# opendilab/LightZero

Measured on NVIDIA H100. Metric: MCTS simulations/sec (batched search+infer), higher is better.
Workload: dtype f32 (fp16x2-split tensor MMAs, fp32 accumulate)

## Files before the change

lightzero_b200/csrc/conv_tc.cu:

```cuda
#include <math.h>
#include <stdlib.h>
#include <string.h>

#include <algorithm>

#include "conv_tc.cuh"
#include "tc_ptx.cuh"

namespace lz {

constexpr int kCvConsumers = 256, kCvThreads = kCvConsumers + 32;
constexpr int kCvStages = 4;

struct CvBars {
    uint64_t full[kCvStages], empty[kCvStages];
    uint64_t in_full;
};

struct CvGeom {
    int nbands, rin, m_lo, mcount, NT, PR;
    size_t plane, part, phase, in_bytes, tap_bytes, smem;
};

__host__ __device__ inline CvGeom cv_geom(const ConvTc &p)
// ... 106 lines not shown
                wg_wait<1>();
                __syncwarp();
                if (lane == 0) mbar_arrive(&bars->empty[(n - 1) % nstages]);
            }
        }
        wg_wait<0>();
        __syncwarp();
        if (lane == 0) mbar_arrive(&bars->empty[(t * 9 + 8) % nstages]);

#pragma unroll
        for (int hr = 0; hr < 2; ++hr) {
            const int m = g.m_lo + t * 128 + wg * 64 + 16 * (warp & 3) + (lane >> 2) + 8 * hr;
            const int k = m / g.rin;
            const int rho = rin0 + (m - k * g.rin);
            const int yy = rho / pitch - 1, xx = rho - (yy + 1) * pitch;
            const bool in_band = (k < nimg) && (rho >= pitch) && (yy >= y0) && (yy < yend);
            const bool valid = in_band && (xx < W);
#pragma unroll
            for (int j = 0; j < N / 8; ++j) {
                const int col = 8 * j + qc;
                const int grp = (N == 128) ? (col >> 6) : 0;
                const int c = col - grp * 64;
                const Tcl &o = p.out[grp];
                const bool relu = p.relu[grp] != 0;
                float v0 = fmaf(acc[4 * j + 2 * hr], __ldg(p.scale + col), __ldg(p.shift + col));
                float v1 = fmaf(acc[4 * j + 2 * hr + 1], __ldg(p.scale + col + 1), __ldg(p.shift + col + 1));
                if (p.res.base && grp == 0 && valid) {
                    const unsigned char *rp = p.res.base + (size_t)(img0 + k) * p.res.img_stride +
                                              ((size_t)(c >> 3) * p.res.plane_rows + rho + 1) * 16 + (c & 7) * 2;
                    const float2 a = __half22float2(*reinterpret_cast<const __half2 *>(rp));
                    const float2 b = __half22float2(*reinterpret_cast<const __half2 *>(rp + p.res.part_stride));
                    v0 += a.x + b.x;
                    v1 += a.y + b.y;
                }
                v0 = valid ? (relu ? fmaxf(v0, 0.0f) : v0) : 0.0f;
                v1 = valid ? (relu ? fmaxf(v1, 0.0f) : v1) : 0.0f;
                if (in_band) {
                    unsigned char *op = o.base + (size_t)(img0 + k) * o.img_stride + ((size_t)(c >> 3) * o.plane_rows + rho + 1) * 16 + (c & 7) * 2;
                    store_split2(op, op + o.part_stride, v0, v1);
                }
            }
        }
    }
}

constexpr int kRbChunks = 16;

struct RbBars {
    uint64_t full[kCvStages], empty[kCvStages];
    uint64_t chunk[kRbChunks];
};

struct RbGeom {
    int nbands, S, m_lo, NT1, NT2, PR, nchunk;
    size_t plane, part, buf, tap_bytes, smem;
};

__host__ __device__ inline RbGeom rb_geom(const ResBlockTc &p)
{
    RbGeom g;
    const int H = p.in.H, pitch = p.in.pitch, kg = p.in.C / 8;
    g.nbands = (H + p.band_h - 1) / p.band_h;
    g.S = (p.band_h + 4) * pitch + 2;
    g.m_lo = pitch + 1;
    g.NT1 = ((p.G - 1) * g.S + (p.band_h + 2) * pitch + 127) / 128;
    g.NT2 = ((p.G - 1) * g.S + p.band_h * pitch + 127) / 128;
    g.PR = p.G * g.S;
    g.nchunk = (g.PR + 127) / 128;
    g.plane = (size_t)g.PR * 16;
    g.part = (size_t)kg * g.plane;
    g.buf = (2 * g.part + 127) & ~(size_t)127;
    g.tap_bytes = (size_t)2 * kg * p.in.C * 16;
    g.smem = 2 * g.buf + p.stages * g.tap_bytes + 1024;
    return g;
}

template <int N>
__device__ __forceinline__ void rb_tiles(float (&acc)[2][N / 2], bool two, uint64_t a_desc0, int row0, const ResBlockTc &p,
                                         const RbGeom &g, uint64_t b_desc0, RbBars *bars, int n0, int lane)
{
    const uint32_t plane16 = (uint32_t)(g.plane >> 4), a_lo16 = (uint32_t)(g.part >> 4), b_lo16 = (uint32_t)N;
    const int nstages = p.stages;
#pragma unroll
    for (int s = 0; s < 2; ++s)
#pragma unroll
        for (int i = 0; i < N / 2; ++i) acc[s][i] = 0.0f;
    for (int tap = 0; tap < 9; ++tap) {
        const int n = n0 + tap, st = n % nstages;
        mbar_wait(&bars->full[st], (n / nstages) & 1);
        const uint64_t b0 = b_desc0 + (uint64_t)((st * g.tap_bytes) >> 4);
        const uint64_t a0 = a_desc0 + (uint64_t)(row0 + p.tap_shift[tap]);
        wg_fence();
        for (int ks = 0; ks < N / 16; ++ks) {
#pragma unroll
            for (int s = 0; s < 2; ++s) {
                if (s == 1 && !two) break;
                const uint64_t as = a0 + s * 128 + ks * 2 * plane16;
                wgmma_f16<N>(acc[s], as, b0 + ks * 4 * N);
                if (p.npass == 3) {
                    wgmma_f16<N>(acc[s], as, b0 + b_lo16 + ks * 4 * N);
                    wgmma_f16<N>(acc[s], as + a_lo16, b0 + ks * 4 * N);
                }
            }
        }
        wg_commit();
        if (tap > 0) {
            wg_wait<1>();
            __syncwarp();
            if (lane == 0) mbar_arrive(&bars->empty[(n - 1) % nstages]);
        }
    }
    wg_wait<0>();
    __syncwarp();
    if (lane == 0) mbar_arrive(&bars->empty[(n0 + 8) % nstages]);
}

template <int N>
__global__ void __launch_bounds__(kCvThreads, 1) k_resblock_tc(ResBlockTc p)
{
    extern __shared__ __align__(1024) unsigned char smem[];
    const RbGeom g = rb_geom(p);
    unsigned char *in_s = smem, *mid_s = smem + g.buf, *ring = smem + 2 * g.buf;
    RbBars *bars = reinterpret_cast<RbBars *>(ring + p.stages * g.tap_bytes);
    const int nstages = p.stages;
    const int tid = threadIdx.x, warp = __shfl_sync(0xffffffffu, tid >> 5, 0), lane = tid & 31;
    const int pitch = p.in.pitch, H = p.in.H, W = p.in.W, kg_in = N / 8;
    const int group = blockIdx.x / g.nbands, band = blockIdx.x - group * g.nbands;
    const int img0 = group * p.G, nimg = min(p.G, p.B - img0);
    const int y0 = band * p.band_h;
    const int np1 = (g.NT1 + 1) / 2, ntaps = 9 * (np1 + (g.NT2 + 1) / 2);

    if (tid == 0) {
        for (int i = 0; i < kCvStages; ++i) { mbar_init(&bars->full[i], 1); mbar_init(&bars->empty[i], kCvConsumers / 32); }
        for (int c = 0; c < g.nchunk; ++c) mbar_init(&bars->chunk[c], 1);
        fence_mbar_init();
    }
    __syncthreads();

    if (warp == kCvConsumers / 32) {
        if (lane == 0) {
            auto load_tap = [&](int n) {
                const int st = n % nstages, tap = n % 9;
                if (n >= nstages) mbar_wait(&bars->empty[st], ((n / nstages) - 1) & 1);
                mbar_expect_tx(&bars->full[st], (uint32_t)g.tap_bytes);
                bulk_g2s(ring + st * g.tap_bytes, p.w[n >= 9 * np1] + (size_t)tap * g.tap_bytes, (uint32_t)g.tap_bytes, &bars->full[st]);
            };
            for (int n = 0; n < nstages; ++n) load_tap(n);
            const int g0 = (y0 - 1) * pitch;
            const int r0 = max(0, -g0), r1 = min(g.S, p.in.plane_rows - g0);
            for (int c = 0; c < g.nchunk; ++c) {
                uint32_t rows = 0;
                for (int k = 0; k < nimg; ++k) rows += (uint32_t)max(0, min(k * g.S + r1, c * 128 + 128) - max(k * g.S + r0, c * 128));
                mbar_expect_tx(&bars->chunk[c], rows * 16u * (uint32_t)(2 * kg_in));
                for (int k = 0; k < nimg; ++k) {
                    const int lo = max(k * g.S + r0, c * 128), hi = min(k * g.S + r1, c * 128 + 128);
                    if (hi <= lo) continue;
                    for (int part = 0; part < 2; ++part)
                        for (int kg = 0; kg < kg_in; ++kg) {
                            const unsigned char *src = p.in.base + (size_t)(img0 + k) * p.in.img_stride + part * p.in.part_stride +
                                                       ((size_t)kg * p.in.plane_rows + g0 + lo - k * g.S) * 16;
                            bulk_g2s(in_s + part * g.part + kg * g.plane + (size_t)lo * 16, src, (uint32_t)(hi - lo) * 16u, &bars->chunk[c]);
                        }
                }
            }
            for (int n = nstages; n < ntaps; ++n) load_tap(n);
        }
        return;
    }

    const int wg = warp >> 2;
    const uint32_t plane16 = (uint32_t)(g.plane >> 4);
    const uint64_t in_desc = make_desc(smem_u32(in_s), plane16, 8), mid_desc = make_desc(smem_u32(mid_s), plane16, 8);
    const uint64_t b_desc0 = make_desc(smem_u32(ring), 2 * N, 8);
    const int qc = 2 * (lane & 3);
    if (tid < 2 * kg_in) *reinterpret_cast<uint4 *>(mid_s + tid * g.plane) = make_uint4(0u, 0u, 0u, 0u);

    int ready = 0;
    for (int t = 0; t < g.NT1; t += 2) {
        const bool two = t + 1 < g.NT1;
        const int need = min(g.nchunk, (t * 128 + 256 + 2 * pitch + 1) / 128 + 1);
        for (; ready < need; ++ready) mbar_wait(&bars->chunk[ready], 0);
        float acc[2][N / 2];
        rb_tiles<N>(acc, two, in_desc, g.m_lo + t * 128 + wg * 64, p, g, b_desc0, bars, t / 2 * 9, lane);
#pragma unroll
        for (int e = 0; e < 4; ++e) {
            const int s = e >> 1, hr = e & 1;
            if (s == 1 && !two) break;
            const int m = g.m_lo + (t + s) * 128 + wg * 64 + 16 * (warp & 3) + (lane >> 2) + 8 * hr;
            const int i = m - pitch;
            const int k = m / g.S;
            const int rho = (y0 - 1) * pitch - 1 + (m - k * g.S);
            const int yy = rho / pitch - 1, xx = rho - (yy + 1) * pitch;
            const bool valid = (k < nimg) && (rho >= pitch) && (yy >= y0 - 1) && (yy <= y0 + p.band_h) && (yy < H) && (xx < W);
            if (i >= g.PR) continue;
#pragma unroll
            for (int j = 0; j < N / 8; ++j) {
                const int col = 8 * j + qc;
                float v0 = fmaf(acc[s][4 * j + 2 * hr], __ldg(p.scale[0] + col), __ldg(p.shift[0] + col));
                float v1 = fmaf(acc[s][4 * j + 2 * hr + 1], __ldg(p.scale[0] + col + 1), __ldg(p.shift[0] + col + 1));
                v0 = valid ? fmaxf(v0, 0.0f) : 0.0f;
                v1 = valid ? fmaxf(v1, 0.0f) : 0.0f;
                unsigned char *op = mid_s + (size_t)(col >> 3) * g.plane + (size_t)i * 16 + (col & 7) * 2;
                store_split2(op, op + g.part, v0, v1);
            }
        }
    }
    for (; ready < g.nchunk; ++ready) mbar_wait(&bars->chunk[ready], 0);
    fence_proxy_async();
    asm volatile("bar.sync 1, %0;\n" ::"n"(kCvConsumers) : "memory");

    const int yend = min(y0 + p.band_h, H);
    for (int t = 0; t < g.NT2; t += 2) {
        const bool two = t + 1 < g.NT2;
        float acc[2][N / 2];
        rb_tiles<N>(acc, two, mid_desc, g.m_lo + t * 128 + wg * 64, p, g, b_desc0, bars, (np1 + t / 2) * 9, lane);
#pragma unroll
        for (int e = 0; e < 4; ++e) {
            const int s = e >> 1, hr = e & 1;
            if (s == 1 && !two) break;
            const int m = g.m_lo + (t + s) * 128 + wg * 64 + 16 * (warp & 3) + (lane >> 2) + 8 * hr;
            const int k = m / g.S;
            const int rho = y0 * pitch - 1 + (m - k * g.S);
            const int yy = rho / pitch - 1, xx = rho - (yy + 1) * pitch;
            const bool in_band = (k < nimg) && (rho >= pitch) && (yy >= y0) && (yy < yend);
            const bool valid = in_band && (xx < W);
            const Tcl &o = p.out;
            size_t obase = 0;
            bool do_write = in_band;
            if (in_band) {
                if (o.nphase == 1) {
                    obase = (size_t)(img0 + k) * o.img_stride + (size_t)(rho + 1) * 16;
                } else if (valid) {
                    const int ph = (yy & 1) * 2 + (xx & 1);
                    const int rho2 = ((yy >> 1) + 1) * o.pitch + (xx >> 1);
                    obase = (size_t)(img0 + k) * o.img_stride + ph * o.phase_stride + (size_t)(rho2 + 1) * 16;
                } else {
                    do_write = false;
                }
            }
#pragma unroll
            for (int j = 0; j < N / 8; ++j) {
                const int col = 8 * j + qc;
                float v0 = fmaf(acc[s][4 * j + 2 * hr], __ldg(p.scale[1] + col), __ldg(p.shift[1] + col));
                float v1 = fmaf(acc[s][4 * j + 2 * hr + 1], __ldg(p.scale[1] + col + 1), __ldg(p.shift[1] + col + 1));
                if (valid) {
                    const unsigned char *rp = in_s + (size_t)(col >> 3) * g.plane + (size_t)(m + pitch) * 16 + (col & 7) * 2;
                    const float2 a = __half22float2(*reinterpret_cast<const __half2 *>(rp));
                    const float2 b = __half22float2(*reinterpret_cast<const __half2 *>(rp + g.part));
                    v0 += a.x + b.x;
                    v1 += a.y + b.y;
                }
                v0 = valid ? fmaxf(v0, 0.0f) : 0.0f;
                v1 = valid ? fmaxf(v1, 0.0f) : 0.0f;
                if (do_write) {
                    unsigned char *op = o.base + obase + (size_t)(col >> 3) * o.plane_rows * 16 + (col & 7) * 2;
                    store_split2(op, op + o.part_stride, v0, v1);
                }
            }
        }
    }
}

__device__ __forceinline__ void tcl_load8(const Tcl &t, int img, int kg, int rho, float (&v)[8])
{
    const unsigned char *pp = t.base + (size_t)img * t.img_stride + ((size_t)kg * t.plane_rows + rho + 1) * 16;
    const uint4 rh = __ldg(reinterpret_cast<const uint4 *>(pp));
    const uint4 rl = __ldg(reinterpret_cast<const uint4 *>(pp + t.part_stride));
    const __half2 *hh = reinterpret_cast<const __half2 *>(&rh), *hl = reinterpret_cast<const __half2 *>(&rl);
#pragma unroll
    for (int j = 0; j < 4; ++j) {
        const float2 a = __half22float2(hh[j]), b = __half22float2(hl[j]);
        v[2 * j] = a.x + b.x;
        v[2 * j + 1] = a.y + b.y;
    }
}

__global__ void k_pool_tcl(Tcl in, Tcl out, float *out_nchw, int B, int Hout)
{
    const int kgs = in.C / 8;
    const size_t n = (size_t)B * kgs * Hout * Hout;
    for (size_t i = blockIdx.x * (size_t)blockDim.x + threadIdx.x; i < n; i += (size_t)gridDim.x * blockDim.x) {
        const int xo = (int)(i % Hout), yo = (int)((i / Hout) % Hout);
        const int kg = (int)((i / ((size_t)Hout * Hout)) % kgs), img = (int)(i / ((size_t)Hout * Hout * kgs));
        float s[8];
#pragma unroll
        for (int j = 0; j < 8; ++j) s[j] = 0.0f;
#pragma unroll
        for (int ky = 0; ky < 3; ++ky) {
            const int yy = 2 * yo + ky - 1;
            if (yy < 0 || yy >= in.H) continue;
#pragma unroll
            for (int kx = 0; kx < 3; ++kx) {
                const int xx = 2 * xo + kx - 1;
                if (xx < 0 || xx >= in.W) continue;
                float v[8];
                tcl_load8(in, img, kg, (yy + 1) * in.pitch + xx, v);
#pragma unroll
                for (int j = 0; j < 8; ++j) s[j] += v[j];
            }
        }
#pragma unroll
        for (int j = 0; j < 8; ++j) s[j] = s[j] / 9.0f;
        if (out_nchw) {
#pragma unroll
            for (int j = 0; j < 8; ++j) out_nchw[((size_t)img * in.C + kg * 8 + j) * Hout * Hout + yo * Hout + xo] = s[j];
        } else {
            unsigned char *op = out.base + (size_t)img * out.img_stride + ((size_t)kg * out.plane_rows + (yo + 1) * out.pitch + xo + 1) * 16;
            store_split8(op, op + out.part_stride, s);
        }
    }
}

int conv_tc_prepare_launch()
{
    const int big = 227 * 1024;
    LZ_CUDA_CHECK(cudaFuncSetAttribute(k_conv_tc<64>, cudaFuncAttributeMaxDynamicSharedMemorySize, big));
    LZ_CUDA_CHECK(cudaFuncSetAttribute(k_conv_tc<128>, cudaFuncAttributeMaxDynamicSharedMemorySize, big));
    LZ_CUDA_CHECK(cudaFuncSetAttribute(k_resblock_tc<32>, cudaFuncAttributeMaxDynamicSharedMemorySize, big));
    LZ_CUDA_CHECK(cudaFuncSetAttribute(k_resblock_tc<64>, cudaFuncAttributeMaxDynamicSharedMemorySize, big));
    return LZ_OK;
}

int conv_tc_launch(const ConvTc &p, cudaStream_t s)
{
    const CvGeom g = cv_geom(p);
    LZ_REQUIRE(g.smem <= 227 * 1024, LZ_EINVAL, "conv_tc: band needs %zu B shared memory", g.smem);
    LZ_REQUIRE(g.tap_bytes <= 16384 && (p.in.C % 16) == 0, LZ_EINVAL, "conv_tc: unsupported channel counts");
    LZ_REQUIRE(p.out[0].nphase == 1 && (p.N < 128 || p.out[1].nphase == 1), LZ_EINVAL, "conv_tc: phase-split output is not supported");
    const int groups = (p.B + p.G - 1) / p.G;
    const int grid = groups * g.nbands;
    switch (p.N) {
        case 64: k_conv_tc<64><<<grid, kCvThreads, g.smem, s>>>(p); break;
        case 128: k_conv_tc<128><<<grid, kCvThreads, g.smem, s>>>(p); break;
        default: LZ_REQUIRE(false, LZ_EINVAL, "conv_tc: N must be 64 or 128");
    }
    LZ_KERNEL_CHECK();
    return LZ_OK;
}

int resblock_tc_plan(ResBlockTc &p)
{
    const int H = p.in.H, W = p.in.W;
    ResBlockTc q = p;
    double best = -1.0;
    for (int G = 1; G <= 4; ++G)
        for (int bh = (G > 1 ? H : 1); bh <= H; ++bh)
            for (int st = 2; st <= 4; st += 2) {
                q.G = G; q.band_h = bh; q.stages = st;
                const RbGeom g = rb_geom(q);
                if (g.smem > 227 * 1024 || g.nchunk > kRbChunks) continue;
                double score = (double)(2 * G * H * W) / ((double)g.nbands * (g.NT1 + g.NT2) * 128);
                score *= (st == 4) ? 1.0 : 0.97;
                if (score > best + 1e-9) { best = score; p.G = G; p.band_h = bh; p.stages = st; }
            }
    LZ_REQUIRE(best > 0.0, LZ_EINVAL, "resblock_tc: no band of a %dx%d, %d-channel block fits shared memory", H, W, p.in.C);
    return LZ_OK;
}

int resblock_tc_launch(const ResBlockTc &p, cudaStream_t s)
{
    const RbGeom g = rb_geom(p);
    LZ_REQUIRE(g.smem <= 227 * 1024 && g.nchunk <= kRbChunks, LZ_EINVAL, "resblock_tc: band needs %zu B shared memory", g.smem);
    LZ_REQUIRE(p.in.nphase == 1 && p.out.C == p.in.C, LZ_EINVAL, "resblock_tc: unsupported input / output layout");
    const int grid = (p.B + p.G - 1) / p.G * g.nbands;
    switch (p.in.C) {
        case 32: k_resblock_tc<32><<<grid, kCvThreads, g.smem, s>>>(p); break;
        case 64: k_resblock_tc<64><<<grid, kCvThreads, g.smem, s>>>(p); break;
        default: LZ_REQUIRE(false, LZ_EINVAL, "resblock_tc: channels must be 32 or 64");
    }
    LZ_KERNEL_CHECK();
    return LZ_OK;
}

size_t conv_tc_packed_bytes(int cin, int ncols) { return (size_t)9 * 2 * (cin / 8) * ncols * 16; }

float conv_tc_pack(const float *w, int cin, int cout, int ncols, int col0, unsigned char *dst)
{
    float mx = 0.0f;
    for (size_t i = 0; i < (size_t)cout * cin * 9; ++i) mx = std::max(mx, fabsf(w[i]));
    int e = 0;
    if (mx > 0.0f) frexpf(mx, &e);
    const float scale = ldexpf(1.0f, 13 - e);
    const size_t tap_halves = (size_t)2 * (cin / 8) * ncols * 8, part_halves = (size_t)ncols * 8;
    __half *h = reinterpret_cast<__half *>(dst);
    for (int t = 0; t < 9; ++t)
        for (int co = 0; co < cout; ++co)
            for (int ci = 0; ci < cin; ++ci) {
                const float sv = w[((size_t)co * cin + ci) * 9 + t] * scale;
                const __half hi = __float2half_rn(sv);
                const __half lo = __float2half_rn(sv - __half2float(hi));
                const size_t off = (size_t)t * tap_halves + ((size_t)(ci / 8) * 2 * ncols + col0 + co) * 8 + (ci % 8);
                h[off] = hi;
                h[off + part_halves] = lo;
            }
    return scale;
}

int pool_tcl_launch(const Tcl &in, const Tcl &out, int B, cudaStream_t s)
{
    const size_t n = (size_t)B * (in.C / 8) * out.H * out.W;
    k_pool_tcl<<<(int)std::min<size_t>((n + 255) / 256, kNumSMs * 32), 256, 0, s>>>(in, out, nullptr, B, out.H);
    LZ_KERNEL_CHECK();
    return LZ_OK;
}

int pool_tcl_to_nchw_launch(const Tcl &in, float *out, int B, int Hout, cudaStream_t s)
{
    const size_t n = (size_t)B * (in.C / 8) * Hout * Hout;
    Tcl dummy = in;
    k_pool_tcl<<<(int)std::min<size_t>((n + 255) / 256, kNumSMs * 32), 256, 0, s>>>(in, dummy, out, B, Hout);
    LZ_KERNEL_CHECK();
    return LZ_OK;
}

}
```

lightzero_b200/csrc/conv_tc.cuh:

```cuda
#pragma once
#include "lz_common.cuh"

namespace lz {

struct Tcl {
    unsigned char *base;
    size_t img_stride, phase_stride, part_stride;
    int plane_rows;
    int C, H, W, pitch;
    int nphase;
};

inline Tcl make_tcl(unsigned char *base, int C, int H, int W, int nphase)
{
    Tcl t;
    t.base = base; t.C = C; t.H = H; t.W = W; t.pitch = W + 1; t.nphase = nphase;
    t.plane_rows = (H + 2) * (W + 1) + 2;
    t.part_stride = (size_t)(C / 8) * t.plane_rows * 16;
    t.phase_stride = 2 * t.part_stride;
    t.img_stride = t.phase_stride * nphase;
    return t;
}
inline size_t tcl_bytes(int B, int C, int H, int W, int nphase)
{
    return (size_t)B * nphase * 2 * (C / 8) * ((size_t)(H + 2) * (W + 1) + 2) * 16;
}

struct ConvTc {
    Tcl in;
    Tcl out[2];
    Tcl res;
    const unsigned char *w;
    const float *scale, *shift;
    int tap_phase[9], tap_shift[9];
    int relu[2];
    int N;
    int G, band_h;
    int stages;
    int B, npass;
};

struct ResBlockTc {
    Tcl in;
    Tcl out;
    const unsigned char *w[2];
    const float *scale[2], *shift[2];
    int tap_shift[9];
    int G, band_h;
    int stages;
    int B, npass;
};

int conv_tc_prepare_launch();
int conv_tc_launch(const ConvTc &p, cudaStream_t s);
int resblock_tc_plan(ResBlockTc &p);
int resblock_tc_launch(const ResBlockTc &p, cudaStream_t s);
float conv_tc_pack(const float *w_torch, int cin, int cout, int ncols, int col0, unsigned char *dst);
size_t conv_tc_packed_bytes(int cin, int ncols);

int pool_tcl_launch(const Tcl &in, const Tcl &out, int B, cudaStream_t s);
int pool_tcl_to_nchw_launch(const Tcl &in, float *out, int B, int Hout, cudaStream_t s);

}
```

lightzero_b200/csrc/model.cu:

```cuda
#include <math.h>
#include <string.h>

#include <algorithm>

#include "model.cuh"
#include "tc_ptx.cuh"

namespace lz {

constexpr int kActFloats = kC * kP;
constexpr int kHFlatMax = 16 * kP;
constexpr int kKpad = 608;

template <int W>
__device__ __forceinline__ void heads_and_outputs(const NetDev &net, float *actA, float *actB, float *hrew,
                                                  float *wstage, bool with_reward, int B, float *o_reward,
                                                  float *o_value, float *o_policy, float *o_reward_logits,
                                                  float *o_value_logits)
{
    const int w = threadIdx.x >> 5, lane = threadIdx.x & 31;
    const int A = net.A, Apad = (A + 31) & ~31;
    float *lg_rew = actB;
    float *lg_val = actB + W * kKpad;
    float *lg_pol = actB + 2 * W * kKpad;
// ... 667 lines not shown
    if (!fold_bn(m, fc + ".1", hid, s2, t2)) return false;
    for (int j = 0; j < hid; ++j) t2[j] += s2[j] * (*B0)[j];
    const int nin = hc * Pix;
    std::vector<float> fc1((size_t)nin * hid), fc2((size_t)hid * K);
    for (int j = 0; j < hid; ++j)
        for (int i = 0; i < nin; ++i) fc1[(size_t)i * hid + j] = (*W0)[(size_t)j * nin + i];
    for (int k = 0; k < K; ++k)
        for (int j = 0; j < hid; ++j) fc2[(size_t)j * K + k] = (*W3)[(size_t)k * hid + j];
    o.w1 = P.add(*w1); o.s1 = P.add(s1); o.t1 = P.add(t1); o.fc1 = P.add(fc1);
    o.s2 = P.add(s2); o.t2 = P.add(t2); o.fc2 = P.add(fc2); o.b2 = P.add(*B3);
    o.hc = hc; o.hid = hid; o.K = K;
    return true;
}

static int pack_tower_tc(lz_model *m)
{
    const std::string R = "representation_network.downsample_net.";
    const int c2 = kC / 2;
    const int h1 = m->tower[0].hout, h2 = m->tower[3].hout, h3 = (h2 - 1) / 2 + 1;
    struct Item { std::string w, bn; int cin, cout; };
    const Item items[9] = {
        {R + "resblocks1.0.conv1.0.weight", R + "resblocks1.0.conv1.1", c2, c2},
        {R + "resblocks1.0.conv2.0.weight", R + "resblocks1.0.conv2.1", c2, c2},
        {R + "downsample_block.conv1.0.weight", R + "downsample_block.conv1.1", c2, kC},
        {R + "downsample_block.conv3.0.weight", "", c2, kC},
        {R + "downsample_block.conv2.0.weight", R + "downsample_block.conv2.1", kC, kC},
        {R + "resblocks2.0.conv1.0.weight", R + "resblocks2.0.conv1.1", kC, kC},
        {R + "resblocks2.0.conv2.0.weight", R + "resblocks2.0.conv2.1", kC, kC},
        {R + "resblocks3.0.conv1.0.weight", R + "resblocks3.0.conv1.1", kC, kC},
        {R + "resblocks3.0.conv2.0.weight", R + "resblocks3.0.conv2.1", kC, kC},
    };
    struct Lay { int it0, it1, cin, N; };
    const Lay lays[8] = {{0, -1, c2, c2}, {1, -1, c2, c2}, {2, 3, c2, 2 * kC}, {4, -1, kC, kC},
                         {5, -1, kC, kC}, {6, -1, kC, kC}, {7, -1, kC, kC}, {8, -1, kC, kC}};
    size_t wbytes = 0;
    for (const Lay &l : lays) wbytes += conv_tc_packed_bytes(l.cin, l.N);
    size_t tab_off = (wbytes + 255) & ~(size_t)255;
    std::vector<unsigned char> host(tab_off + 8 * 2 * 128 * sizeof(float), 0);
    float *tab = reinterpret_cast<float *>(host.data() + tab_off);
    size_t woff[8], off = 0;
    for (int li = 0; li < 8; ++li) {
        const Lay &l = lays[li];
        woff[li] = off;
        float *scale = tab + li * 256, *shift = scale + 128;
        for (int part = 0; part < 2; ++part) {
            const int it = part == 0 ? l.it0 : l.it1;
            if (it < 0) continue;
            const Item &I = items[it];
            auto w = find(m, I.w, (size_t)I.cout * I.cin * 9);
            if (!w) return LZ_EINVAL;
            std::vector<float> sc(I.cout, 1.0f), sh(I.cout, 0.0f);
            if (!I.bn.empty() && !fold_bn(m, I.bn, I.cout, sc, sh)) return LZ_EINVAL;
            const int col0 = part * kC;
            const float ws = conv_tc_pack(w->data(), I.cin, I.cout, l.N, col0, host.data() + off);
            for (int k = 0; k < I.cout; ++k) { scale[col0 + k] = sc[k] / ws; shift[col0 + k] = sh[k]; }
        }
        off += conv_tc_packed_bytes(l.cin, l.N);
    }
    if (m->d_tower) cudaFree(m->d_tower);
    m->d_tower = nullptr;
    int rc = dev_alloc(&m->d_tower, host.size());
    if (rc != LZ_OK) return rc;
    LZ_CUDA_CHECK(cudaMemcpy(m->d_tower, host.data(), host.size(), cudaMemcpyHostToDevice));
    const float *dtab = reinterpret_cast<const float *>(m->d_tower + tab_off);
    auto base = [&](int li, int N, int H, int nphase_in, int C_in) {
        ConvTc p;
        memset(&p, 0, sizeof(p));
        p.w = m->d_tower + woff[li];
        p.scale = dtab + li * 256; p.shift = p.scale + 128;
        p.N = N; p.relu[0] = 1; p.relu[1] = 0;
        p.in = make_tcl(nullptr, C_in, H, H, nphase_in);
        for (int t = 0; t < 9; ++t) {
            const int ky = t / 3, kx = t % 3;
            if (nphase_in == 1) { p.tap_phase[t] = 0; p.tap_shift[t] = (ky - 1) * p.in.pitch + (kx - 1); }
            else {
                p.tap_phase[t] = (((ky + 1) & 1) * 2) + ((kx + 1) & 1);
                p.tap_shift[t] = (ky == 0 ? -p.in.pitch : 0) + (kx == 0 ? -1 : 0);
            }
        }
        pick_band(p);
        return p;
    };
    m->tower_tc[0] = base(2, 2 * kC, h2, 4, c2);
    m->tower_tc[1] = base(3, kC, h2, 1, kC);
    auto block = [&](ResBlockTc &p, int li, int C, int H) {
        memset(&p, 0, sizeof(p));
        for (int c = 0; c < 2; ++c) {
            p.w[c] = m->d_tower + woff[li + c];
            p.scale[c] = dtab + (li + c) * 256; p.shift[c] = p.scale[c] + 128;
        }
        p.in = make_tcl(nullptr, C, H, H, 1);
        for (int t = 0; t < 9; ++t) p.tap_shift[t] = (t / 3 - 1) * p.in.pitch + (t % 3 - 1);
        return resblock_tc_plan(p);
    };
    if ((rc = block(m->tower_rb[0], 0, c2, h1))) return rc;
    if ((rc = block(m->tower_rb[1], 4, kC, h2))) return rc;
    if ((rc = block(m->tower_rb[2], 6, kC, h3))) return rc;
    return conv_tc_prepare_launch();
}

static int pack_tc(lz_model *m, const NetDev &net)
{
    const lz_model_config &c = m->cfg;
    const int A = c.action_space_size, n = c.num_res_blocks;
    const int nconv = 1 + 6 * n;
    const size_t conv_bytes = (size_t)tc_conv_layout_bytes();
    const size_t off_convw = 0;
// ... 458 lines not shown
```

lightzero_b200/csrc/tc_ptx.cuh:

```cuda
#pragma once
#include <cuda_fp16.h>
#include <cuda_runtime.h>
#include <stdint.h>
#include <stdio.h>

namespace lz {

__device__ __forceinline__ uint32_t smem_u32(const void *p) { return (uint32_t)__cvta_generic_to_shared(p); }

__device__ __forceinline__ void mbar_init(uint64_t *bar, uint32_t count)
{
    asm volatile("mbarrier.init.shared::cta.b64 [%0], %1;\n" ::"r"(smem_u32(bar)), "r"(count));
}
__device__ __forceinline__ void mbar_arrive(uint64_t *bar)
{
    asm volatile("{\n\t.reg .b64 st;\n\tmbarrier.arrive.shared::cta.b64 st, [%0];\n\t}\n" ::"r"(smem_u32(bar)) : "memory");
}
__device__ __forceinline__ void mbar_expect_tx(uint64_t *bar, uint32_t bytes)
{
    asm volatile("{\n\t.reg .b64 st;\n\tmbarrier.arrive.expect_tx.shared::cta.b64 st, [%0], %1;\n\t}\n" ::"r"(smem_u32(bar)), "r"(bytes) : "memory");
}
__device__ __forceinline__ void mbar_wait(uint64_t *bar, uint32_t parity)
{
    const uint32_t a = smem_u32(bar);
// ... 6 lines not shown
    asm volatile("trap;\n");
}
__device__ __forceinline__ void bulk_g2s(void *dst, const void *src, uint32_t bytes, uint64_t *bar)
{
    asm volatile("cp.async.bulk.shared::cluster.global.mbarrier::complete_tx::bytes [%0], [%1], %2, [%3];\n"
                 ::"r"(smem_u32(dst)), "l"(src), "r"(bytes), "r"(smem_u32(bar)) : "memory");
}
__device__ __forceinline__ void fence_proxy_async() { asm volatile("fence.proxy.async.shared::cta;\n" ::: "memory"); }
__device__ __forceinline__ void fence_mbar_init() { asm volatile("fence.mbarrier_init.release.cluster;\n" ::: "memory"); }

__device__ __forceinline__ void wg_fence() { asm volatile("wgmma.fence.sync.aligned;\n" ::: "memory"); }
__device__ __forceinline__ void wg_commit() { asm volatile("wgmma.commit_group.sync.aligned;\n" ::: "memory"); }
template <int N>
__device__ __forceinline__ void wg_wait() { asm volatile("wgmma.wait_group.sync.aligned %0;\n" ::"n"(N) : "memory"); }

template <int N>
__device__ __forceinline__ void wg_fence_acc(float (&d)[N])
{
#pragma unroll
    for (int i = 0; i < N; ++i) asm volatile("" : "+f"(d[i])::"memory");
}

#define LZ_WG_R8(o) "+f"(d[o + 0]), "+f"(d[o + 1]), "+f"(d[o + 2]), "+f"(d[o + 3]), "+f"(d[o + 4]), "+f"(d[o + 5]), "+f"(d[o + 6]), "+f"(d[o + 7])
__device__ __forceinline__ void wgmma_n16(float (&d)[8], uint64_t a, uint64_t b)
{
    asm volatile("{\n\t.reg .pred p;\n\tsetp.ne.b32 p, 1, 0;\n\t"
                 "wgmma.mma_async.sync.aligned.m64n16k16.f32.f16.f16 {%0, %1, %2, %3, %4, %5, %6, %7}, %8, %9, p, 1, 1, 0, 0;\n\t}\n"
                 : LZ_WG_R8(0) : "l"(a), "l"(b));
}
__device__ __forceinline__ void wgmma_n32(float (&d)[16], uint64_t a, uint64_t b)
{
    asm volatile("{\n\t.reg .pred p;\n\tsetp.ne.b32 p, 1, 0;\n\t"
                 "wgmma.mma_async.sync.aligned.m64n32k16.f32.f16.f16 {%0, %1, %2, %3, %4, %5, %6, %7, %8, %9, %10, %11, %12, %13, %14, "
                 "%15}, %16, %17, p, 1, 1, 0, 0;\n\t}\n"
                 : LZ_WG_R8(0), LZ_WG_R8(8) : "l"(a), "l"(b));
}
__device__ __forceinline__ void wgmma_n64(float (&d)[32], uint64_t a, uint64_t b)
{
    asm volatile("{\n\t.reg .pred p;\n\tsetp.ne.b32 p, 1, 0;\n\t"
                 "wgmma.mma_async.sync.aligned.m64n64k16.f32.f16.f16 {%0, %1, %2, %3, %4, %5, %6, %7, %8, %9, %10, %11, %12, %13, %14, "
                 "%15, %16, %17, %18, %19, %20, %21, %22, %23, %24, %25, %26, %27, %28, %29, %30, %31}, %32, %33, p, 1, 1, 0, 0;\n\t}\n"
                 : LZ_WG_R8(0), LZ_WG_R8(8), LZ_WG_R8(16), LZ_WG_R8(24) : "l"(a), "l"(b));
}
__device__ __forceinline__ void wgmma_n128(float (&d)[64], uint64_t a, uint64_t b)
{
    asm volatile("{\n\t.reg .pred p;\n\tsetp.ne.b32 p, 1, 0;\n\t"
                 "wgmma.mma_async.sync.aligned.m64n128k16.f32.f16.f16 {%0, %1, %2, %3, %4, %5, %6, %7, %8, %9, %10, %11, %12, %13, %14, "
                 "%15, %16, %17, %18, %19, %20, %21, %22, %23, %24, %25, %26, %27, %28, %29, %30, %31, %32, %33, %34, %35, %36, %37, %38, "
                 "%39, %40, %41, %42, %43, %44, %45, %46, %47, %48, %49, %50, %51, %52, %53, %54, %55, %56, %57, %58, %59, %60, %61, %62, "
                 "%63}, %64, %65, p, 1, 1, 0, 0;\n\t}\n"
                 : LZ_WG_R8(0), LZ_WG_R8(8), LZ_WG_R8(16), LZ_WG_R8(24), LZ_WG_R8(32), LZ_WG_R8(40), LZ_WG_R8(48), LZ_WG_R8(56)
                 : "l"(a), "l"(b));
}
#undef LZ_WG_R8
template <int N>
__device__ __forceinline__ void wgmma_f16(float (&d)[N / 2], uint64_t a, uint64_t b)
{
    if constexpr (N == 16) wgmma_n16(d, a, b);
    else if constexpr (N == 32) wgmma_n32(d, a, b);
    else if constexpr (N == 64) wgmma_n64(d, a, b);
    else wgmma_n128(d, a, b);
}

template <int N>
__device__ __forceinline__ void wg_stage(float *S, int ld, int row0, int col0, const float (&d)[N / 2])
{
    const int w = (threadIdx.x >> 5) & 3, lane = threadIdx.x & 31;
    float *p0 = S + (size_t)(row0 + 16 * w + (lane >> 2)) * ld + col0 + 2 * (lane & 3), *p1 = p0 + 8 * ld;
#pragma unroll
    for (int j = 0; j < N / 8; ++j) {
        *reinterpret_cast<float2 *>(p0 + 8 * j) = make_float2(d[4 * j], d[4 * j + 1]);
        *reinterpret_cast<float2 *>(p1 + 8 * j) = make_float2(d[4 * j + 2], d[4 * j + 3]);
    }
}

__device__ __forceinline__ uint64_t make_desc(uint32_t saddr, uint32_t lbo16, uint32_t sbo16)
{
    return (uint64_t)((saddr >> 4) & 0x3FFFu) | ((uint64_t)(lbo16 & 0x3FFFu) << 16) | ((uint64_t)(sbo16 & 0x3FFFu) << 32);
}

__device__ __forceinline__ void store_split8(unsigned char *hi_ptr, unsigned char *lo_ptr, const float *v)
{
    __half2 h[4], l[4];
#pragma unroll
    for (int i = 0; i < 4; ++i) {
        float a = v[2 * i], b = v[2 * i + 1];
        a = fminf(fmaxf(a, -65504.0f), 65504.0f);
        b = fminf(fmaxf(b, -65504.0f), 65504.0f);
        __half ha = __float2half_rn(a), hb = __float2half_rn(b);
        h[i] = __halves2half2(ha, hb);
        l[i] = __halves2half2(__float2half_rn(a - __half2float(ha)), __float2half_rn(b - __half2float(hb)));
    }
    *reinterpret_cast<uint4 *>(hi_ptr) = *reinterpret_cast<uint4 *>(h);
    *reinterpret_cast<uint4 *>(lo_ptr) = *reinterpret_cast<uint4 *>(l);
}


__device__ __forceinline__ void store_split8_pos(unsigned char *hi_ptr, unsigned char *lo_ptr, const float *v)
{
    __half2 h[4], l[4];
#pragma unroll
    for (int i = 0; i < 4; ++i) {
        const float a = fminf(v[2 * i], 65504.0f), b = fminf(v[2 * i + 1], 65504.0f);
        h[i] = __floats2half2_rn(a, b);
        const float2 back = __half22float2(h[i]);
        l[i] = __floats2half2_rn(a - back.x, b - back.y);
    }
    *reinterpret_cast<uint4 *>(hi_ptr) = *reinterpret_cast<uint4 *>(h);
    *reinterpret_cast<uint4 *>(lo_ptr) = *reinterpret_cast<uint4 *>(l);
}

}
```

Baseline: 4.527 million.

## Transpose C=32 resblock GEMM so pixels map to wgmma N=256 dimension

```diff
diff --git a/lightzero_b200/csrc/conv_tc.cu b/lightzero_b200/csrc/conv_tc.cu
--- a/lightzero_b200/csrc/conv_tc.cu
+++ b/lightzero_b200/csrc/conv_tc.cu
@@ -182,7 +182,7 @@
 };
 
 struct RbGeom {
-    int nbands, S, m_lo, NT1, NT2, PR, nchunk;
+    int nbands, S, m_lo, rows1, rows2, tr, NT1, NT2, PR, nchunk;
     size_t plane, part, buf, tap_bytes, smem;
 };
 
@@ -193,8 +193,11 @@
     g.nbands = (H + p.band_h - 1) / p.band_h;
     g.S = (p.band_h + 4) * pitch + 2;
     g.m_lo = pitch + 1;
-    g.NT1 = ((p.G - 1) * g.S + (p.band_h + 2) * pitch + 127) / 128;
-    g.NT2 = ((p.G - 1) * g.S + p.band_h * pitch + 127) / 128;
+    g.rows1 = (p.G - 1) * g.S + (p.band_h + 2) * pitch;
+    g.rows2 = (p.G - 1) * g.S + p.band_h * pitch;
+    g.tr = (p.in.C == 32) ? 256 : 128;
+    g.NT1 = (g.rows1 + g.tr - 1) / g.tr;
+    g.NT2 = (g.rows2 + g.tr - 1) / g.tr;
     g.PR = p.G * g.S;
     g.nchunk = (g.PR + 127) / 128;
     g.plane = (size_t)g.PR * 16;
@@ -205,6 +208,8 @@
     return g;
 }
 
+__host__ __device__ inline int rb_tile_rows(int rows, int t) { return rows - t * 256 <= 128 ? 128 : 256; }
+
 template <int N>
 __device__ __forceinline__ void rb_tiles(float (&acc)[2][N / 2], bool two, uint64_t a_desc0, int row0, const ResBlockTc &p,
                                          const RbGeom &g, uint64_t b_desc0, RbBars *bars, int n0, int lane)
@@ -245,7 +250,110 @@
     if (lane == 0) mbar_arrive(&bars->empty[(n0 + 8) % nstages]);
 }
 
-template <int N>
+__device__ __forceinline__ void rb_tile_t(float (&acc)[128], int n, uint64_t x_desc0, int row0, const ResBlockTc &p, const RbGeom &g,
+                                          uint64_t w_desc0, RbBars *bars, int n0, int lane)
+{
+    const uint32_t plane16 = (uint32_t)(g.plane >> 4), x_lo16 = (uint32_t)(g.part >> 4);
+    float (&acc128)[64] = *reinterpret_cast<float (*)[64]>(&acc[0]);
+    const int nstages = p.stages;
+#pragma unroll
+    for (int i = 0; i < 128; ++i) acc[i] = 0.0f;
+    for (int tap = 0; tap < 9; ++tap) {
+        const int s = n0 + tap, st = s % nstages;
+        mbar_wait(&bars->full[st], (s / nstages) & 1);
+        const uint64_t w0 = w_desc0 + (uint64_t)((st * g.tap_bytes) >> 4);
+        const uint64_t x0 = x_desc0 + (uint64_t)(row0 + p.tap_shift[tap]);
+        wg_fence();
+#pragma unroll
+        for (int ks = 0; ks < 2; ++ks) {
+            const uint64_t a = w0 + ks * 128, b = x0 + ks * 2 * plane16;
+            if (n == 256) {
+                wgmma_n256(acc, a, b);
+                if (p.npass == 3) wgmma_n256(acc, a, b + x_lo16);
+            } else if (n == 128) {
+                wgmma_n128(acc128, a, b);
+                if (p.npass == 3) wgmma_n128(acc128, a, b + x_lo16);
+            }
+        }
+        wg_commit();
+        if (tap > 0) {
+            wg_wait<1>();
+            __syncwarp();
+            if (lane == 0) mbar_arrive(&bars->empty[(s - 1) % nstages]);
+        }
+    }
+    wg_wait<0>();
+    __syncwarp();
+    if (lane == 0) mbar_arrive(&bars->empty[(n0 + 8) % nstages]);
+}
+
+struct RbPix {
+    int k, r, yy, xx;
+    __device__ __forceinline__ void init(int m, int rho_off, int S, int pitch)
+    {
+        k = m / S;
+        r = m - k * S;
+        const int rr = rho_off + r + 2 * pitch;
+        const int q = rr / pitch;
+        xx = rr - q * pitch;
+        yy = q - 3;
+    }
+    __device__ __forceinline__ void step8(int S, int pitch, int band_h)
+    {
+        r += 8;
+        xx += 8;
+        if (xx >= pitch) { xx -= pitch; ++yy; }
+        if (r >= S) {
+            r -= S;
+            ++k;
+            xx -= 2;
+            yy -= band_h + 4;
+            if (xx < 0) { xx += pitch; --yy; }
+        }
+    }
+};
+
+__device__ __forceinline__ void split2(float a, float b, uint32_t &hi, uint32_t &lo)
+{
+    a = fminf(fmaxf(a, -65504.0f), 65504.0f);
+    b = fminf(fmaxf(b, -65504.0f), 65504.0f);
+    const __half ha = __float2half_rn(a), hb = __float2half_rn(b);
+    __half2 h = __halves2half2(ha, hb), l = __halves2half2(__float2half_rn(a - __half2float(ha)), __float2half_rn(b - __half2float(hb)));
+    hi = *reinterpret_cast<uint32_t *>(&h);
+    lo = *reinterpret_cast<uint32_t *>(&l);
+}
+
+template <bool RES, typename Store>
+__device__ __forceinline__ void rb_epilogue_t(const float (&acc)[128], int n, const float *scale, const float *shift, int npass,
+                                              uint32_t res_addr, Store store)
+{
+    const int ch = 8 * ((threadIdx.x >> 5) & 3) + ((threadIdx.x & 31) >> 2);
+    const float sc = __ldg(scale + ch), sh = __ldg(shift + ch);
+#pragma unroll
+    for (int j = 0; j < 32; ++j) {
+        if (8 * j >= n) break;
+        float v[2];
+#pragma unroll
+        for (int e = 0; e < 2; ++e) {
+            float a = acc[4 * j + e];
+            if (npass == 3) a += acc[4 * j + 2 + e];
+            v[e] = fmaf(a, sc, sh);
+        }
+        if constexpr (RES) {
+            uint32_t r[2];
+            ldmatrix_x2_trans(r, res_addr + j * 128);
+            const float2 a = __half22float2(*reinterpret_cast<const __half2 *>(&r[0]));
+            const float2 b = __half22float2(*reinterpret_cast<const __half2 *>(&r[1]));
+            v[0] += a.x + b.x;
+            v[1] += a.y + b.y;
+        }
+        uint32_t hi, lo;
+        split2(fmaxf(v[0], 0.0f), fmaxf(v[1], 0.0f), hi, lo);
+        store(j, movmatrix_trans(hi), movmatrix_trans(lo));
+    }
+}
+
+template <int C>
 __global__ void __launch_bounds__(kCvThreads, 1) k_resblock_tc(ResBlockTc p)
 {
     extern __shared__ __align__(1024) unsigned char smem[];
@@ -254,7 +362,7 @@
     RbBars *bars = reinterpret_cast<RbBars *>(ring + p.stages * g.tap_bytes);
     const int nstages = p.stages;
     const int tid = threadIdx.x, warp = __shfl_sync(0xffffffffu, tid >> 5, 0), lane = tid & 31;
-    const int pitch = p.in.pitch, H = p.in.H, W = p.in.W, kg_in = N / 8;
+    const int pitch = p.in.pitch, H = p.in.H, W = p.in.W, kg_in = C / 8;
     const int group = blockIdx.x / g.nbands, band = blockIdx.x - group * g.nbands;
     const int img0 = group * p.G, nimg = min(p.G, p.B - img0);
     const int y0 = band * p.band_h;
@@ -298,93 +406,156 @@
         return;
     }
 
-    const int wg = warp >> 2;
+    const int wg = warp >> 2, w = warp & 3;
     const uint32_t plane16 = (uint32_t)(g.plane >> 4);
     const uint64_t in_desc = make_desc(smem_u32(in_s), plane16, 8), mid_desc = make_desc(smem_u32(mid_s), plane16, 8);
-    const uint64_t b_desc0 = make_desc(smem_u32(ring), 2 * N, 8);
+    const uint64_t w_desc0 = make_desc(smem_u32(ring), 2 * C, 8);
     const int qc = 2 * (lane & 3);
+    const int yend = min(y0 + p.band_h, H);
+    const Tcl &o = p.out;
     if (tid < 2 * kg_in) *reinterpret_cast<uint4 *>(mid_s + tid * g.plane) = make_uint4(0u, 0u, 0u, 0u);
-
     int ready = 0;
-    for (int t = 0; t < g.NT1; t += 2) {
-        const bool two = t + 1 < g.NT1;
-        const int need = min(g.nchunk, (t * 128 + 256 + 2 * pitch + 1) / 128 + 1);
-        for (; ready < need; ++ready) mbar_wait(&bars->chunk[ready], 0);
-        float acc[2][N / 2];
-        rb_tiles<N>(acc, two, in_desc, g.m_lo + t * 128 + wg * 64, p, g, b_desc0, bars, t / 2 * 9, lane);
-#pragma unroll
-        for (int e = 0; e < 4; ++e) {
-            const int s = e >> 1, hr = e & 1;
-            if (s == 1 && !two) break;
-            const int m = g.m_lo + (t + s) * 128 + wg * 64 + 16 * (warp & 3) + (lane >> 2) + 8 * hr;
-            const int i = m - pitch;
-            const int k = m / g.S;
-            const int rho = (y0 - 1) * pitch - 1 + (m - k * g.S);
-            const int yy = rho / pitch - 1, xx = rho - (yy + 1) * pitch;
-            const bool valid = (k < nimg) && (rho >= pitch) && (yy >= y0 - 1) && (yy <= y0 + p.band_h) && (yy < H) && (xx < W);
-            if (i >= g.PR) continue;
-#pragma unroll
-            for (int j = 0; j < N / 8; ++j) {
-                const int col = 8 * j + qc;
-                float v0 = fmaf(acc[s][4 * j + 2 * hr], __ldg(p.scale[0] + col), __ldg(p.shift[0] + col));
-                float v1 = fmaf(acc[s][4 * j + 2 * hr + 1], __ldg(p.scale[0] + col + 1), __ldg(p.shift[0] + col + 1));
-                v0 = valid ? fmaxf(v0, 0.0f) : 0.0f;
-                v1 = valid ? fmaxf(v1, 0.0f) : 0.0f;
-                unsigned char *op = mid_s + (size_t)(col >> 3) * g.plane + (size_t)i * 16 + (col & 7) * 2;
-                store_split2(op, op + g.part, v0, v1);
-            }
-        }
-    }
-    for (; ready < g.nchunk; ++ready) mbar_wait(&bars->chunk[ready], 0);
-    fence_proxy_async();
-    asm volatile("bar.sync 1, %0;\n" ::"n"(kCvConsumers) : "memory");
-
-    const int yend = min(y0 + p.band_h, H);
-    for (int t = 0; t < g.NT2; t += 2) {
-        const bool two = t + 1 < g.NT2;
-        float acc[2][N / 2];
-        rb_tiles<N>(acc, two, mid_desc, g.m_lo + t * 128 + wg * 64, p, g, b_desc0, bars, (np1 + t / 2) * 9, lane);
-#pragma unroll
-        for (int e = 0; e < 4; ++e) {
-            const int s = e >> 1, hr = e & 1;
-            if (s == 1 && !two) break;
-            const int m = g.m_lo + (t + s) * 128 + wg * 64 + 16 * (warp & 3) + (lane >> 2) + 8 * hr;
-            const int k = m / g.S;
-            const int rho = y0 * pitch - 1 + (m - k * g.S);
-            const int yy = rho / pitch - 1, xx = rho - (yy + 1) * pitch;
-            const bool in_band = (k < nimg) && (rho >= pitch) && (yy >= y0) && (yy < yend);
-            const bool valid = in_band && (xx < W);
-            const Tcl &o = p.out;
-            size_t obase = 0;
-            bool do_write = in_band;
-            if (in_band) {
-                if (o.nphase == 1) {
-                    obase = (size_t)(img0 + k) * o.img_stride + (size_t)(rho + 1) * 16;
-                } else if (valid) {
-                    const int ph = (yy & 1) * 2 + (xx & 1);
-                    const int rho2 = ((yy >> 1) + 1) * o.pitch + (xx >> 1);
-                    obase = (size_t)(img0 + k) * o.img_stride + ph * o.phase_stride + (size_t)(rho2 + 1) * 16;
-                } else {
-                    do_write = false;
-                }
-            }
-#pragma unroll
-            for (int j = 0; j < N / 8; ++j) {
-                const int col = 8 * j + qc;
-                float v0 = fmaf(acc[s][4 * j + 2 * hr], __ldg(p.scale[1] + col), __ldg(p.shift[1] + col));
-                float v1 = fmaf(acc[s][4 * j + 2 * hr + 1], __ldg(p.scale[1] + col + 1), __ldg(p.shift[1] + col + 1));
-                if (valid) {
-                    const unsigned char *rp = in_s + (size_t)(col >> 3) * g.plane + (size_t)(m + pitch) * 16 + (col & 7) * 2;
-                    const float2 a = __half22float2(*reinterpret_cast<const __half2 *>(rp));
-                    const float2 b = __half22float2(*reinterpret_cast<const __half2 *>(rp + g.part));
-                    v0 += a.x + b.x;
-                    v1 += a.y + b.y;
-                }
-                v0 = valid ? fmaxf(v0, 0.0f) : 0.0f;
-                v1 = valid ? fmaxf(v1, 0.0f) : 0.0f;
+
+    if constexpr (C == 32) {
+        for (int t = wg; t < 2 * np1; t += 2) {
+            const int n = t < g.NT1 ? rb_tile_rows(g.rows1, t) : 0;
+            const int m0 = g.m_lo + t * 256;
+            const int need = min(g.nchunk, (m0 + n + pitch) / 128 + 1);
+            if (n) for (; ready < need; ++ready) mbar_wait(&bars->chunk[ready], 0);
+            float acc[128];
+            rb_tile_t(acc, n, in_desc, m0, p, g, w_desc0, bars, (t >> 1) * 9, lane);
+            if (!n) continue;
+            RbPix px;
+            px.init(m0 + (lane >> 2), (y0 - 1) * pitch - 1, g.S, pitch);
+            const int ylo = max(y0 - 1, 0), yhi = min(y0 + p.band_h, H - 1);
+            rb_epilogue_t<false>(acc, n, p.scale[0], p.shift[0], p.npass, 0u, [&](int j, uint32_t hi, uint32_t lo) {
+                const bool valid = (px.k < nimg) && (px.yy >= ylo) && (px.yy <= yhi) && (px.xx < W);
+                int i = m0 + 8 * j + (lane >> 2) - pitch;
+                if (i >= g.PR) i = 0;
+                unsigned char *op = mid_s + (size_t)w * g.plane + (size_t)i * 16 + qc * 2;
+                *reinterpret_cast<uint32_t *>(op) = valid ? hi : 0u;
+                *reinterpret_cast<uint32_t *>(op + g.part) = valid ? lo : 0u;
+                px.step8(g.S, pitch, p.band_h);
+            });
+        }
+        for (; ready < g.nchunk; ++ready) mbar_wait(&bars->chunk[ready], 0);
+        fence_proxy_async();
+        asm volatile("bar.sync 1, %0;\n" ::"n"(kCvConsumers) : "memory");
+
+        const int rpart = (lane >> 3) & 1;
+        for (int t = wg; t < 2 * ((g.NT2 + 1) / 2); t += 2) {
+            const int n = t < g.NT2 ? rb_tile_rows(g.rows2, t) : 0;
+            const int m0 = g.m_lo + t * 256;
+            float acc[128];
+            rb_tile_t(acc, n, mid_desc, m0, p, g, w_desc0, bars, (np1 + (t >> 1)) * 9, lane);
+            if (!n) continue;
+            RbPix px;
+            px.init(m0 + (lane >> 2), y0 * pitch - 1, g.S, pitch);
+            const uint32_t res_addr = smem_u32(in_s + rpart * g.part + (size_t)w * g.plane + (size_t)(m0 + pitch + (lane & 7)) * 16);
+            rb_epilogue_t<true>(acc, n, p.scale[1], p.shift[1], p.npass, res_addr, [&](int j, uint32_t hi, uint32_t lo) {
+                const bool in_band = (px.k < nimg) && (px.yy >= y0) && (px.yy < yend);
+                const bool valid = in_band && (px.xx < W);
+                const int rho = (px.yy + 1) * pitch + px.xx;
+                size_t obase = 0;
+                bool do_write = in_band;
+                if (in_band) {
+                    if (o.nphase == 1) {
+                        obase = (size_t)(img0 + px.k) * o.img_stride + (size_t)(rho + 1) * 16;
+                    } else if (valid) {
+                        const int ph = (px.yy & 1) * 2 + (px.xx & 1);
+                        const int rho2 = ((px.yy >> 1) + 1) * o.pitch + (px.xx >> 1);
+                        obase = (size_t)(img0 + px.k) * o.img_stride + ph * o.phase_stride + (size_t)(rho2 + 1) * 16;
+                    } else {
+                        do_write = false;
+                    }
+                }
                 if (do_write) {
-                    unsigned char *op = o.base + obase + (size_t)(col >> 3) * o.plane_rows * 16 + (col & 7) * 2;
-                    store_split2(op, op + o.part_stride, v0, v1);
+                    unsigned char *op = o.base + obase + (size_t)w * o.plane_rows * 16 + qc * 2;
+                    *reinterpret_cast<uint32_t *>(op) = valid ? hi : 0u;
+                    *reinterpret_cast<uint32_t *>(op + o.part_stride) = valid ? lo : 0u;
+                }
+                px.step8(g.S, pitch, p.band_h);
+            });
+        }
+    } else {
+        for (int t = 0; t < g.NT1; t += 2) {
+            const bool two = t + 1 < g.NT1;
+            const int need = min(g.nchunk, (t * 128 + 256 + 2 * pitch + 1) / 128 + 1);
+            for (; ready < need; ++ready) mbar_wait(&bars->chunk[ready], 0);
+            float acc[2][C / 2];
+            rb_tiles<C>(acc, two, in_desc, g.m_lo + t * 128 + wg * 64, p, g, w_desc0, bars, t / 2 * 9, lane);
+#pragma unroll
+            for (int e = 0; e < 4; ++e) {
+                const int s = e >> 1, hr = e & 1;
+                if (s == 1 && !two) break;
+                const int m = g.m_lo + (t + s) * 128 + wg * 64 + 16 * w + (lane >> 2) + 8 * hr;
+                const int i = m - pitch;
+                const int k = m / g.S;
+                const int rho = (y0 - 1) * pitch - 1 + (m - k * g.S);
+                const int yy = rho / pitch - 1, xx = rho - (yy + 1) * pitch;
+                const bool valid = (k < nimg) && (rho >= pitch) && (yy >= y0 - 1) && (yy <= y0 + p.band_h) && (yy < H) && (xx < W);
+                if (i >= g.PR) continue;
+#pragma unroll
+                for (int j = 0; j < C / 8; ++j) {
+                    const int col = 8 * j + qc;
+                    float v0 = fmaf(acc[s][4 * j + 2 * hr], __ldg(p.scale[0] + col), __ldg(p.shift[0] + col));
+                    float v1 = fmaf(acc[s][4 * j + 2 * hr + 1], __ldg(p.scale[0] + col + 1), __ldg(p.shift[0] + col + 1));
+                    v0 = valid ? fmaxf(v0, 0.0f) : 0.0f;
+                    v1 = valid ? fmaxf(v1, 0.0f) : 0.0f;
+                    unsigned char *op = mid_s + (size_t)(col >> 3) * g.plane + (size_t)i * 16 + (col & 7) * 2;
+                    store_split2(op, op + g.part, v0, v1);
+                }
+            }
+        }
+        for (; ready < g.nchunk; ++ready) mbar_wait(&bars->chunk[ready], 0);
+        fence_proxy_async();
+        asm volatile("bar.sync 1, %0;\n" ::"n"(kCvConsumers) : "memory");
+
+        for (int t = 0; t < g.NT2; t += 2) {
+            const bool two = t + 1 < g.NT2;
+            float acc[2][C / 2];
+            rb_tiles<C>(acc, two, mid_desc, g.m_lo + t * 128 + wg * 64, p, g, w_desc0, bars, (np1 + t / 2) * 9, lane);
+#pragma unroll
+            for (int e = 0; e < 4; ++e) {
+                const int s = e >> 1, hr = e & 1;
+                if (s == 1 && !two) break;
+                const int m = g.m_lo + (t + s) * 128 + wg * 64 + 16 * w + (lane >> 2) + 8 * hr;
+                const int k = m / g.S;
+                const int rho = y0 * pitch - 1 + (m - k * g.S);
+                const int yy = rho / pitch - 1, xx = rho - (yy + 1) * pitch;
+                const bool in_band = (k < nimg) && (rho >= pitch) && (yy >= y0) && (yy < yend);
+                const bool valid = in_band && (xx < W);
+                size_t obase = 0;
+                bool do_write = in_band;
+                if (in_band) {
+                    if (o.nphase == 1) {
+                        obase = (size_t)(img0 + k) * o.img_stride + (size_t)(rho + 1) * 16;
+                    } else if (valid) {
+                        const int ph = (yy & 1) * 2 + (xx & 1);
+                        const int rho2 = ((yy >> 1) + 1) * o.pitch + (xx >> 1);
+                        obase = (size_t)(img0 + k) * o.img_stride + ph * o.phase_stride + (size_t)(rho2 + 1) * 16;
+                    } else {
+                        do_write = false;
+                    }
+                }
+#pragma unroll
+                for (int j = 0; j < C / 8; ++j) {
+                    const int col = 8 * j + qc;
+                    float v0 = fmaf(acc[s][4 * j + 2 * hr], __ldg(p.scale[1] + col), __ldg(p.shift[1] + col));
+                    float v1 = fmaf(acc[s][4 * j + 2 * hr + 1], __ldg(p.scale[1] + col + 1), __ldg(p.shift[1] + col + 1));
+                    if (valid) {
+                        const unsigned char *rp = in_s + (size_t)(col >> 3) * g.plane + (size_t)(m + pitch) * 16 + (col & 7) * 2;
+                        const float2 a = __half22float2(*reinterpret_cast<const __half2 *>(rp));
+                        const float2 b = __half22float2(*reinterpret_cast<const __half2 *>(rp + g.part));
+                        v0 += a.x + b.x;
+                        v1 += a.y + b.y;
+                    }
+                    v0 = valid ? fmaxf(v0, 0.0f) : 0.0f;
+                    v1 = valid ? fmaxf(v1, 0.0f) : 0.0f;
+                    if (do_write) {
+                        unsigned char *op = o.base + obase + (size_t)(col >> 3) * o.plane_rows * 16 + (col & 7) * 2;
+                        store_split2(op, op + o.part_stride, v0, v1);
+                    }
                 }
             }
         }
@@ -468,6 +639,11 @@
     return LZ_OK;
 }
 
+static int rb_issued_rows(const RbGeom &g, int rows, int nt)
+{
+    return g.tr == 128 ? nt * 128 : (nt - 1) * 256 + rb_tile_rows(rows, nt - 1);
+}
+
 int resblock_tc_plan(ResBlockTc &p)
 {
     const int H = p.in.H, W = p.in.W;
@@ -479,7 +655,9 @@
                 q.G = G; q.band_h = bh; q.stages = st;
                 const RbGeom g = rb_geom(q);
                 if (g.smem > 227 * 1024 || g.nchunk > kRbChunks) continue;
-                double score = (double)(2 * G * H * W) / ((double)g.nbands * (g.NT1 + g.NT2) * 128);
+                if ((size_t)(g.m_lo + g.NT2 * g.tr + p.in.pitch + 2 - g.PR) * 16 > st * g.tap_bytes) continue;
+                const int issued = rb_issued_rows(g, g.rows1, g.NT1) + rb_issued_rows(g, g.rows2, g.NT2);
+                double score = (double)(2 * G * H * W) / ((double)g.nbands * issued);
                 score *= (st == 4) ? 1.0 : 0.97;
                 if (score > best + 1e-9) { best = score; p.G = G; p.band_h = bh; p.stages = st; }
             }
@@ -491,7 +669,7 @@
 {
     const RbGeom g = rb_geom(p);
     LZ_REQUIRE(g.smem <= 227 * 1024 && g.nchunk <= kRbChunks, LZ_EINVAL, "resblock_tc: band needs %zu B shared memory", g.smem);
-    LZ_REQUIRE(p.in.nphase == 1 && p.out.C == p.in.C, LZ_EINVAL, "resblock_tc: unsupported input / output layout");
+    LZ_REQUIRE(p.in.nphase == 1 && p.out.C == p.in.C && p.in.W >= 8, LZ_EINVAL, "resblock_tc: unsupported input / output layout");
     const int grid = (p.B + p.G - 1) / p.G * g.nbands;
     switch (p.in.C) {
         case 32: k_resblock_tc<32><<<grid, kCvThreads, g.smem, s>>>(p); break;
@@ -504,14 +682,14 @@
 
 size_t conv_tc_packed_bytes(int cin, int ncols) { return (size_t)9 * 2 * (cin / 8) * ncols * 16; }
 
-float conv_tc_pack(const float *w, int cin, int cout, int ncols, int col0, unsigned char *dst)
+float conv_tc_pack(const float *w, int cin, int cout, int ncols, int col0, unsigned char *dst, bool interleave)
 {
     float mx = 0.0f;
     for (size_t i = 0; i < (size_t)cout * cin * 9; ++i) mx = std::max(mx, fabsf(w[i]));
     int e = 0;
     if (mx > 0.0f) frexpf(mx, &e);
     const float scale = ldexpf(1.0f, 13 - e);
-    const size_t tap_halves = (size_t)2 * (cin / 8) * ncols * 8, part_halves = (size_t)ncols * 8;
+    const size_t tap_halves = (size_t)2 * (cin / 8) * ncols * 8;
     __half *h = reinterpret_cast<__half *>(dst);
     for (int t = 0; t < 9; ++t)
         for (int co = 0; co < cout; ++co)
@@ -519,9 +697,12 @@
                 const float sv = w[((size_t)co * cin + ci) * 9 + t] * scale;
                 const __half hi = __float2half_rn(sv);
                 const __half lo = __float2half_rn(sv - __half2float(hi));
-                const size_t off = (size_t)t * tap_halves + ((size_t)(ci / 8) * 2 * ncols + col0 + co) * 8 + (ci % 8);
+                const int col = col0 + co;
+                const int row_hi = interleave ? (col / 8) * 16 + (col % 8) : col;
+                const int lo_rows = interleave ? 8 : ncols;
+                const size_t off = (size_t)t * tap_halves + ((size_t)(ci / 8) * 2 * ncols + row_hi) * 8 + (ci % 8);
                 h[off] = hi;
-                h[off + part_halves] = lo;
+                h[off + (size_t)lo_rows * 8] = lo;
             }
     return scale;
 }
diff --git a/lightzero_b200/csrc/conv_tc.cuh b/lightzero_b200/csrc/conv_tc.cuh
--- a/lightzero_b200/csrc/conv_tc.cuh
+++ b/lightzero_b200/csrc/conv_tc.cuh
@@ -55,7 +55,7 @@
 int conv_tc_launch(const ConvTc &p, cudaStream_t s);
 int resblock_tc_plan(ResBlockTc &p);
 int resblock_tc_launch(const ResBlockTc &p, cudaStream_t s);
-float conv_tc_pack(const float *w_torch, int cin, int cout, int ncols, int col0, unsigned char *dst);
+float conv_tc_pack(const float *w_torch, int cin, int cout, int ncols, int col0, unsigned char *dst, bool interleave);
 size_t conv_tc_packed_bytes(int cin, int ncols);
 
 int pool_tcl_launch(const Tcl &in, const Tcl &out, int B, cudaStream_t s);
diff --git a/lightzero_b200/csrc/model.cu b/lightzero_b200/csrc/model.cu
--- a/lightzero_b200/csrc/model.cu
+++ b/lightzero_b200/csrc/model.cu
@@ -743,7 +743,7 @@
             std::vector<float> sc(I.cout, 1.0f), sh(I.cout, 0.0f);
             if (!I.bn.empty() && !fold_bn(m, I.bn, I.cout, sc, sh)) return LZ_EINVAL;
             const int col0 = part * kC;
-            const float ws = conv_tc_pack(w->data(), I.cin, I.cout, l.N, col0, host.data() + off);
+            const float ws = conv_tc_pack(w->data(), I.cin, I.cout, l.N, col0, host.data() + off, li <= 1);
             for (int k = 0; k < I.cout; ++k) { scale[col0 + k] = sc[k] / ws; shift[col0 + k] = sh[k]; }
         }
         off += conv_tc_packed_bytes(l.cin, l.N);
diff --git a/lightzero_b200/csrc/tc_ptx.cuh b/lightzero_b200/csrc/tc_ptx.cuh
--- a/lightzero_b200/csrc/tc_ptx.cuh
+++ b/lightzero_b200/csrc/tc_ptx.cuh
@@ -82,6 +82,21 @@
                  : LZ_WG_R8(0), LZ_WG_R8(8), LZ_WG_R8(16), LZ_WG_R8(24), LZ_WG_R8(32), LZ_WG_R8(40), LZ_WG_R8(48), LZ_WG_R8(56)
                  : "l"(a), "l"(b));
 }
+#define LZ_WG_R32(o) LZ_WG_R8(o), LZ_WG_R8(o + 8), LZ_WG_R8(o + 16), LZ_WG_R8(o + 24)
+__device__ __forceinline__ void wgmma_n256(float (&d)[128], uint64_t a, uint64_t b)
+{
+    asm volatile("{\n\t.reg .pred p;\n\tsetp.ne.b32 p, 1, 0;\n\t"
+                 "wgmma.mma_async.sync.aligned.m64n256k16.f32.f16.f16 {"
+                 "%0, %1, %2, %3, %4, %5, %6, %7, %8, %9, %10, %11, %12, %13, %14, %15, %16, %17, %18, %19, %20, %21, %22, %23, "
+                 "%24, %25, %26, %27, %28, %29, %30, %31, %32, %33, %34, %35, %36, %37, %38, %39, %40, %41, %42, %43, %44, %45, %46, "
+                 "%47, %48, %49, %50, %51, %52, %53, %54, %55, %56, %57, %58, %59, %60, %61, %62, %63, %64, %65, %66, %67, %68, %69, "
+                 "%70, %71, %72, %73, %74, %75, %76, %77, %78, %79, %80, %81, %82, %83, %84, %85, %86, %87, %88, %89, %90, %91, %92, "
+                 "%93, %94, %95, %96, %97, %98, %99, %100, %101, %102, %103, %104, %105, %106, %107, %108, %109, %110, %111, %112, "
+                 "%113, %114, %115, %116, %117, %118, %119, %120, %121, %122, %123, %124, %125, %126, %127}, %128, %129, p, 1, 1, 0, 0;\n\t}\n"
+                 : LZ_WG_R32(0), LZ_WG_R32(32), LZ_WG_R32(64), LZ_WG_R32(96)
+                 : "l"(a), "l"(b));
+}
+#undef LZ_WG_R32
 #undef LZ_WG_R8
 template <int N>
 __device__ __forceinline__ void wgmma_f16(float (&d)[N / 2], uint64_t a, uint64_t b)
@@ -102,6 +117,17 @@
         *reinterpret_cast<float2 *>(p0 + 8 * j) = make_float2(d[4 * j], d[4 * j + 1]);
         *reinterpret_cast<float2 *>(p1 + 8 * j) = make_float2(d[4 * j + 2], d[4 * j + 3]);
     }
+}
+
+__device__ __forceinline__ void ldmatrix_x2_trans(uint32_t (&r)[2], uint32_t saddr)
+{
+    asm volatile("ldmatrix.sync.aligned.m8n8.x2.trans.shared.b16 {%0, %1}, [%2];\n" : "=r"(r[0]), "=r"(r[1]) : "r"(saddr) : "memory");
+}
+__device__ __forceinline__ uint32_t movmatrix_trans(uint32_t x)
+{
+    uint32_t y;
+    asm volatile("movmatrix.sync.aligned.m8n8.trans.b16 %0, %1;\n" : "=r"(y) : "r"(x));
+    return y;
 }
 
 __device__ __forceinline__ uint64_t make_desc(uint32_t saddr, uint32_t lbo16, uint32_t sbo16)
```

New measurement: 4.589 million (median of 6 runs). No clear change (+1.4%).
